# arneschneuing/DiffSBDD

Measured on AMD Instinct MI355X. Metric: sampled ligands/sec (500-step DDPM, fullatom_cond) at 1/2/4/8 MI355X, higher is better.
Workload: dtype f32

## Files before the change

diffsbdd_amd/csrc/edge_mlp.h:

```cpp
#pragma once
#include "common.h"

namespace dsbdd {

struct EdgeMlpW {
  const float* P;
  const float* Q;
  const float* wd;
  const float* wd0;
  const float* table;
  const float* W2T;
  const float* b2;
  const float* W2TP;
  const float* W2TP16;
  const void* W2E;
  const float* W2SK;
};

__global__ void permute_w2t_kernel(const float* src, float* dst, int H) {
  const int i = blockIdx.x * blockDim.x + threadIdx.x;
  if (i >= H * H) return;
  const int k = i / H, o = i % H, ct = H / 32;
  const int j = o / ct, c = o % ct;
  dst[i] = src[k * H + c * 32 + j];
// ... 62 lines not shown
  const int row = (blockIdx.x * kThreads + threadIdx.x) >> 6, lane = threadIdx.x & 63;
  if (row >= n_rows + n_ghost) return;
  const bool ghost = row >= n_rows;
  const int da = ghost ? 0 : deg_a[row], sa = ghost ? 0 : row_ptr_a[row];
  const int a0 = sa >> 5, a1 = min((sa + da - 1) >> 5, max_tile);
  int db = 0, sb = 0, tw = 0;
  if (row >= n_lig) {
    const int tl = ghost ? row - n_rows : twin_local[row - n_lig];
    db = deg_b[tl]; sb = row_ptr_b[tl]; tw = twin_base + tl;
  }
  const int b0 = sb >> 5, b1 = min((sb + db - 1) >> 5, max_tile);
  for (int k = 4 * lane; k < H; k += 256) {
    float4 v = make_float4(0.f, 0.f, 0.f, 0.f);
    if (da > 0) {
      v = ld4(agg + (size_t)row * H + k);
      for (int T = a0 + 1; T <= a1; ++T) {
        const float4 h = ld4(head_a + (size_t)T * H + k);
        v.x += h.x; v.y += h.y; v.z += h.z; v.w += h.w;
      }
    }
    if (db > 0) {
      float4 u = ld4(agg_b + (size_t)tw * H + k);
      for (int T = b0 + 1; T <= b1; ++T) {
        const float4 h = ld4(head_b + (size_t)T * H + k);
        u.x += h.x; u.y += h.y; u.z += h.z; u.w += h.w;
      }
      v.x += u.x; v.y += u.y; v.z += u.z; v.w += u.w;
    }
    *reinterpret_cast<float4*>(agg + (size_t)row * H + k) = v;
  }
}


__global__ __launch_bounds__(kThreads) void agg_complete_shell_kernel(
    float* agg, const float* agg_head, const int* row_ptr, const int* deg, int n_rows, int H, int max_tile,
    const int* lvl, int shell_level, int n_lig, int n_nodes, const float* head_s, const int* sh_ptr, const int* sh_deg,
    const int* row_ptr_nat, const int* ecol_nat, int e_cap_nat, const int* twin_local, const int* row_ptr_ghost,
    const float* msg, int msg_slots, float inv_norm) {
  const int row = (blockIdx.x * kThreads + threadIdx.x) >> 6, lane = threadIdx.x & 63;
  if (row >= n_rows) return;
  const int L = (row >= n_lig && row < n_nodes) ? lvl[row] : 0;
  if (L > shell_level) return;
  if (L < shell_level) {
    const int d = deg[row], s = row_ptr[row];
    const int t0 = s >> 5, t1 = min((s + d - 1) >> 5, max_tile);
    if (d > 0 && t1 == t0) return;
    for (int k = 4 * lane; k < H; k += 256) {
      float4 v = make_float4(0.f, 0.f, 0.f, 0.f);
      if (d > 0) {
        v = ld4(agg + (size_t)row * H + k);
        for (int T = t0 + 1; T <= t1; ++T) {
          const float4 h = ld4(agg_head + (size_t)T * H + k);
          v.x += h.x; v.y += h.y; v.z += h.z; v.w += h.w;
        }
      }
      *reinterpret_cast<float4*>(agg + (size_t)row * H + k) = v;
    }
    return;
  }
  const int d = sh_deg[row], s = sh_ptr[row];
  const int t0 = s >> 5, t1 = min((s + d - 1) >> 5, max_tile);
  const int dn = deg[row], sn = row_ptr_nat[row];
  const int e_lo = max(sn, 0), e_hi = min(sn + dn, e_cap_nat);
  const int base = row_ptr_ghost[twin_local[row - n_lig]] - sn;
  const int k = min(4 * lane, H - 4);
  const bool on = 4 * lane < H;
  float4 v = make_float4(0.f, 0.f, 0.f, 0.f);
  if (d > 0 && on) {
    v = ld4(agg + (size_t)row * H + k);
    for (int T = t0 + 1; T <= t1; ++T) {
      const float4 h = ld4(head_s + (size_t)T * H + k);
      v.x += h.x; v.y += h.y; v.z += h.z; v.w += h.w;
    }
  }
  float4 c = make_float4(0.f, 0.f, 0.f, 0.f);
  for (int e0 = e_lo; e0 < e_hi; e0 += 64) {
    const int e = e0 + lane;
    bool take = false;
    if (e < e_hi) {
      const int j = ecol_nat[e];
      take = (unsigned)j < (unsigned)n_nodes && j >= n_lig && lvl[j] >= shell_level &&
             (unsigned)(base + e) < (unsigned)msg_slots;
    }
    unsigned long long mk = __ballot(take);
    while (mk) {
      const float* src[4];
      int n = 0;
#pragma unroll
      for (int u = 0; u < 4; ++u)
        if (mk) {
          src[n++] = msg + (size_t)(base + e0 + (__ffsll((long long)mk) - 1)) * H + k;
          mk &= mk - 1;
        }
      float4 m[4];
#pragma unroll
      for (int u = 0; u < 4; ++u) if (u < n) m[u] = ld4(src[u]);
#pragma unroll
      for (int u = 0; u < 4; ++u) if (u < n) { c.x += m[u].x; c.y += m[u].y; c.z += m[u].z; c.w += m[u].w; }
    }
  }
  v.x += c.x * inv_norm; v.y += c.y * inv_norm; v.z += c.z * inv_norm; v.w += c.w * inv_norm;
  if (on) *reinterpret_cast<float4*>(agg + (size_t)row * H + k) = v;
}

}
```

diffsbdd_amd/csrc/engine.hip:

```cpp
#include "../../include/diffsbdd_hip.h"

#include <algorithm>
#include <climits>
#include <cmath>
#include <cstdio>
#include <cstdlib>
#include <cstring>
#include <string>
#include <type_traits>
#include <utility>
#include <vector>

#include "common.h"
#include "ddpm.h"
#include "edge_mlp.h"
#include "edge_wave.h"
#include "edge_wave16.h"
#include "edge_splitk.h"
#include "graph_parts.h"
#include "radius_graph.h"
#include "level_list.h"
#include "geometry.h"
#include "lig_head.h"
#include "ligand_pack.h"
// ... 229 lines not shown
  double tot = 0.0;
  for (size_t i = 0; i + 1 < e->ev_used; i += 2) {
    HIP_TRY(hipEventSynchronize(e->ev[i + 1]));
    float ms = 0.f;
    HIP_TRY(hipEventElapsedTime(&ms, e->ev[i], e->ev[i + 1]));
    tot += ms;
  }
  *total_ms = tot;
  *launches = (int64_t)(e->ev_used / 2);
  e->ev_used = 0;
  return DSBDD_OK;
}

int dsbdd_engine_graph_stats(const dsbdd_engine* e, int64_t* replays, int64_t* captures, int64_t* eager) {
  if (!e || !replays || !captures || !eager) return fail(DSBDD_ERR_ARG, "null argument");
  *replays = e->n_replay; *captures = e->n_capture; *eager = e->n_eager;
  return DSBDD_OK;
}

int dsbdd_engine_buffer(const dsbdd_engine* e, int which, void** out) {
  if (!e || !out || !e->ws) return fail(DSBDD_ERR_STATE, "no workspace bound");
  void* const buf[] = {e->erow, e->ecol, e->ed0, e->row_ptr, e->h, e->x, e->node_batch, e->deg, e->lvl, e->lvl_list, e->lvl_cnt,
                       e->lvl_end, e->row_ptrL, e->erowL, e->ecolL, e->ed0L, e->lvl_stats};
  static_assert(DSBDD_BUF_LEVEL_STATS + 1 == sizeof(buf) / sizeof(buf[0]), "one pointer per DSBDD_BUF_* id");
  if (which < 0 || which > DSBDD_BUF_LEVEL_STATS) return fail(DSBDD_ERR_ARG, "unknown buffer id");
  *out = buf[which];
  return DSBDD_OK;
}

int dsbdd_engine_list2_read(const dsbdd_engine* e, int which, void* dst, int64_t count) {
  if (!e || !dst || count < 0) return fail(DSBDD_ERR_ARG, "bad argument");
  if (!e->ws) return fail(DSBDD_ERR_STATE, "no workspace bound");
  const int64_t N = e->cap_lig + e->cap_poc;
  const int* src = which == DSBDD_LIST2_DEG ? e->deg2 : (which == DSBDD_LIST2_ROW_PTR ? e->row_ptr2 : nullptr);
  if (!src) return fail(DSBDD_ERR_ARG, "unknown list-2 buffer");
  if (count > N + (which == DSBDD_LIST2_ROW_PTR ? 1 : 0)) return fail(DSBDD_ERR_CAPACITY, "list-2 read past the buffer");
  HIP_TRY(hipDeviceSynchronize());
  HIP_TRY(hipMemcpy(dst, src, (size_t)count * 4, hipMemcpyDeviceToHost));
  return DSBDD_OK;
}

int dsbdd_engine_shell_read(const dsbdd_engine* e, int which, int list, void* dst, int64_t count) {
  if (!e || !dst || count < 0) return fail(DSBDD_ERR_ARG, "bad argument");
  if (!e->shell_mem) return fail(DSBDD_ERR_STATE, "no shell stage has run on this engine");
  const int64_t N = e->shell_key[0], SL = e->shell_key[2];
  const void* src = nullptr;
  int64_t have = 0, size = 4;
  const bool lst = list >= 0 && list < kShellLists;
  switch (which) {
    case DSBDD_SHELL_STATS: src = e->sh_stats; have = 8; size = 8; break;
    case DSBDD_SHELL_COUNT: src = e->sh_cnt; have = kShellLists; break;
    case DSBDD_SHELL_ROW: if (lst) { src = e->sh_row + (size_t)list * SL; have = SL; } break;
    case DSBDD_SHELL_COL: if (lst) { src = e->sh_col + (size_t)list * SL; have = SL; } break;
    case DSBDD_SHELL_PTR: src = e->sh_ptr; have = N; break;
    case DSBDD_SHELL_DEG: src = e->sh_deg; have = N; break;
  }
  if (!src) return fail(DSBDD_ERR_ARG, "unknown shell buffer");
  if (count > have) return fail(DSBDD_ERR_CAPACITY, "shell read past the buffer");
  HIP_TRY(hipDeviceSynchronize());
  HIP_TRY(hipMemcpy(dst, src, (size_t)(count * size), hipMemcpyDeviceToHost));
  return DSBDD_OK;
}

int dsbdd_dynamics_forward(dsbdd_engine* e, void* stream, const float* xh_lig, const float* xh_pocket,
                           const float* t, int64_t t_count, const int64_t* mask_lig,
                           const int64_t* mask_pocket, int64_t n_lig, int64_t n_pocket, int64_t batch,
                           const int32_t* ext_row, const int32_t* ext_col, int64_t ext_n_edges,
                           float* eps_lig, float* eps_pocket, int32_t* status) {
  StreamDevice stream_device_(stream);
  if (!e || !xh_lig || !xh_pocket || !t || !mask_lig || !mask_pocket || !eps_lig || !status)
    return fail(DSBDD_ERR_ARG, "null argument");
  if (!e->has_weights) return fail(DSBDD_ERR_STATE, "weights not set");
  if (!e->ws) return fail(DSBDD_ERR_STATE, "workspace not bound");
  if (n_lig > e->cap_lig || n_pocket > e->cap_poc || batch > e->cap_batch || n_lig < 0 || n_pocket < 0 ||
      batch < 1)
    return fail(DSBDD_ERR_CAPACITY, "sizes exceed the bound workspace");
  if (t_count != 1 && t_count != batch) return fail(DSBDD_ERR_ARG, "t must have 1 or batch entries");
  if (ext_row && (!ext_col || ext_n_edges < 0 || ext_n_edges > e->cap_edges))
    return fail(DSBDD_ERR_CAPACITY, "external edge list exceeds edge capacity");
  hipStream_t s = static_cast<hipStream_t>(stream);
  const ForwardArgs args{xh_lig, xh_pocket, t, t_count, mask_lig, mask_pocket, n_lig, n_pocket, batch,
                         ext_row, ext_col, ext_n_edges, eps_lig, eps_pocket, status};
  const int rc = frame_upkeep(e, s, args);
  if (rc) return rc;
  e->time_now = e->profile > 0 && (e->prof_call++ % e->profile) == 0;
  if (!e->use_graph || e->time_now || e->trace_h || e->trace_x || ext_row) {
    ++e->n_eager;
    return forward_impl(e, s, args);
// ... 6 lines not shown
```

diffsbdd_amd/csrc/graph_parts.h:

```cpp
#pragma once
#include "common.h"

namespace dsbdd {

constexpr int kTileCtrInts = 32;
constexpr int kEdgeAlign = 32;
constexpr int kLevels = 5;
constexpr int kShellLists = 2;

__host__ __device__ __forceinline__ int align_edges(int v) { return (v + kEdgeAlign - 1) & ~(kEdgeAlign - 1); }

template <class I>
__device__ __forceinline__ int lower_bound_i64(const I* a, int n, long long v) {
  static_assert(sizeof(I) == 8, "64-bit masks");
  int lo = 0, hi = n;
  while (lo < hi) {
    const int mid = (lo + hi) >> 1;
    if (a[mid] < v) lo = mid + 1; else hi = mid;
  }
  return lo;
}

struct SampleRows {
  int l0, l1, p0, p1;
// ... 65 lines not shown
    const int idx = lo + lane * step;
    const int c = __popcll(__ballot(idx < hi && a[idx] < v));
    if (c == 0) return lo;
    const int last = lo + (c - 1) * step;
    hi = min(last + step, hi);
    lo = last + 1;
  }
  return lo;
}

__device__ __forceinline__ SampleRows sample_rows_wg(const int64_t* mask_lig, int n_lig, const int64_t* mask_poc,
                                                     int n_poc, int b, int* s_rows) {
  static_assert(kThreads == 256, "one wave per bound");
  const int w = threadIdx.x >> 6, lane = threadIdx.x & 63;
  const int r = w < 2 ? lower_bound_wave(mask_lig, n_lig, b + (w & 1), lane)
                      : lower_bound_wave(mask_poc, n_poc, b + (w & 1), lane);
  if (lane == 0) s_rows[w] = r;
  __syncthreads();
  return SampleRows{s_rows[0], s_rows[1], s_rows[2], s_rows[3]};
}

__device__ __forceinline__ void sample_mean_body(const float* x, const int* lig_off, const int* poc_off, int n_lig,
                                                 float* mean, float (*red)[kThreads]) {
  const int b = blockIdx.x, t = threadIdx.x;
  const SampleRows r = sample_rows(lig_off, poc_off, n_lig, b);
  float s0 = 0.f, s1 = 0.f, s2 = 0.f;
  for (int i = r.l0 + t; i < r.l1; i += kThreads) { s0 += x[3 * i]; s1 += x[3 * i + 1]; s2 += x[3 * i + 2]; }
  for (int i = r.p0 + t; i < r.p1; i += kThreads) { s0 += x[3 * i]; s1 += x[3 * i + 1]; s2 += x[3 * i + 2]; }
  block_sum3(s0, s1, s2, red);
  if (t < 3) mean[3 * b + t] = red[t][0] / (float)r.count();
  __syncthreads();
}

__device__ __forceinline__ int pad_fill(int from, int lane, int* erow, int* ecol, float* ed0, int cap) {
  const int to = align_edges(from), pos = from + lane;
  if (pos >= 0 && pos < to && pos < cap) { erow[pos] = -1; ecol[pos] = 0; ed0[pos] = 0.f; }
  return to;
}

__global__ void zero_kernel(uint4* p, size_t n16, unsigned char* tail, int n_tail) {
  const uint4 z = make_uint4(0u, 0u, 0u, 0u);
  for (size_t i = blockIdx.x * (size_t)blockDim.x + threadIdx.x; i < n16; i += (size_t)gridDim.x * blockDim.x)
    p[i] = z;
  if (blockIdx.x == 0 && (int)threadIdx.x < n_tail) tail[threadIdx.x] = 0;
}

inline hipError_t zero_async(void* ptr, size_t bytes, hipStream_t s) {
  if (bytes == 0) return hipSuccess;
  const size_t n16 = bytes / 16;
  const int n_tail = (int)(bytes % 16);
  size_t blocks = (n16 + 255) / 256;
  if (blocks > 2048) blocks = 2048;
  if (blocks < 1) blocks = 1;
  hipLaunchKernelGGL(zero_kernel, dim3((unsigned)blocks), dim3(256), 0, s, static_cast<uint4*>(ptr), n16,
                     static_cast<unsigned char*>(ptr) + n16 * 16, n_tail);
  return hipGetLastError();
}

}
```

diffsbdd_amd/csrc/launch.h:

```cpp
#pragma once

static hipError_t nl(hipStream_t s, const float* A1, int lda1, int K1, const float* A2, int lda2, int K2,
                     const float* WT, int ldw, const float* bias, const float* R, int ldr, float* C,
                     int ldc, int64_t M, int N, int act) {
  NodeLinearArgs a{A1, lda1, K1, A2, lda2, K2, WT, ldw, bias, R, ldr, C, ldc, (int)M, N, act, nullptr, nullptr};
  return launch_node_linear(s, a);
}

template <class... P, class... A>
static int launch_1d(void (*kernel)(P...), size_t n_items, hipStream_t s, A... args) {
  hipLaunchKernelGGL(kernel, dim3((unsigned)((n_items + 255) / 256)), dim3(256), 0, s, static_cast<P>(args)...);
  HIP_TRY(hipGetLastError());
  return DSBDD_OK;
}

static int device_cus() {
  static int cache[64] = {0};
  int dev = 0;
  if (hipGetDevice(&dev) != hipSuccess || dev < 0 || dev >= 64) return 256;
  if (cache[dev] == 0) {
    hipDeviceProp_t pr;
    int n = 0;
    if (hipGetDeviceProperties(&pr, dev) == hipSuccess) n = pr.multiProcessorCount;
    cache[dev] = n > 0 ? n : 256;
// ... 88 lines not shown
    a.tail_s = e->tail > 1 ? e->tail : resident;
    grid = persistent_grid((edge_bound + 127) / 128 * 4, e->n_cu, 2, e->edge_max_wg, 8);
  }
  if (a.msg_out) {
    if (mode != MODE_GCL || e->cfg.hidden_nf != 256 || e->emu || !a.mlp[0].W2TP || a.wt_base) return hipErrorInvalidValue;
    hipLaunchKernelGGL((edge_wave_kernel<256, MODE_GCL, true, 0, false, true>), dim3(grid), dim3(kThreads), 0, s, a);
    return hipGetLastError();
  }
  return with_hidden(e->cfg.hidden_nf, [&](auto h) {
    constexpr int H = decltype(h)::value;
    return emu ? launch_wave_emu_t<H>(s, mode, a, grid, emu) : launch_wave_t<H>(s, mode, a, grid);
  });
}

static hipError_t launch_edge_plain(int H, hipStream_t s, int mode, const EdgeArgs& a, int64_t edge_bound) {
  const int grid = edge_wave_grid(mode, a, edge_bound, device_cus(), 0);
  if (a.z2_out && (a.e_count_b || a.wt_base)) return hipErrorInvalidValue;
  return with_hidden(H, [&](auto h) {
    constexpr int HH = decltype(h)::value;
    return a.z2_out ? launch_wave_store_t<HH>(s, mode, a, grid) : launch_wave_t<HH>(s, mode, a, grid);
  });
}

static Cutoffs cutoffs_of(const dsbdd_config& c) {
  return Cutoffs{c.has_cutoff_ligand, c.has_cutoff_pocket, c.has_cutoff_interaction,
                 c.cutoff_ligand, c.cutoff_pocket, c.cutoff_interaction};
}

static int build_edges_impl(hipStream_t s, const float* x, int n_lig, int N, int B, const dsbdd_config& c,
                            const int* node_batch, const int* lig_off, const int* poc_off, int* deg,
                            int* row_ptr, int* erow, int* ecol, float* ed0, int64_t cap, int* status,
                            int* act_flag = nullptr, int* scan_tmp = nullptr, int* seg_base = nullptr,
                            const EdgeList2* list2 = nullptr, int id_offset = 0, int* lvl = nullptr) {
  const int waves_per_block = kThreads / 64;
  int blocks = (N + waves_per_block - 1) / waves_per_block;
  if (blocks > 4096) blocks = 4096;
  if (blocks < 1) blocks = 1;
  const Cutoffs cut = cutoffs_of(c);
  const int aligned = scan_tmp && seg_base;
  SegAlign sg{node_batch, lig_off, poc_off, n_lig, B, scan_tmp, aligned ? seg_base : nullptr};
  EdgeList2 l2{};
  if (list2 && aligned) l2 = *list2;
  hipLaunchKernelGGL((edges_kernel<false>), dim3(blocks), dim3(kThreads), 0, s, x, node_batch, lig_off,
                     poc_off, n_lig, N, cut, deg, (const int*)nullptr, (int*)nullptr, (int*)nullptr,
                     (float*)nullptr, 0, status, act_flag, SegAlign{}, (int*)nullptr, l2, 0, lvl);
  HIP_TRY(hipGetLastError());
  hipLaunchKernelGGL(scan_kernel, dim3(l2.deg ? 2 : 1), dim3(1024), 0, s, (const int*)deg, row_ptr, N, sg,
                     (const int*)l2.deg, l2.row_ptr, l2.seg);
  HIP_TRY(hipGetLastError());
  hipLaunchKernelGGL((edges_kernel<true>), dim3(blocks), dim3(kThreads), 0, s, x, node_batch, lig_off,
                     poc_off, n_lig, N, cut, deg, (const int*)row_ptr, erow, ecol, ed0, (int)cap, status,
                     (int*)nullptr, sg, row_ptr, l2, id_offset, (int*)nullptr);
  HIP_TRY(hipGetLastError());
  return DSBDD_OK;
}
```

diffsbdd_amd/csrc/level_list.h:

```cpp
#pragma once
#include "common.h"
#include "graph_parts.h"

namespace dsbdd {

struct LevelArgs {
  const int* node_batch; const int* lig_off; const int* poc_off; int n_lig; int B;
  int* lvl;
  const int* deg;
  const int* row_ptr_nat;
  const int* erow_nat; const int* ecol_nat; const float* ed0_nat;
  int* seg_rows;
  int* seg_edges;
  int* node_base;
  int* edge_base;
  int* lvl_cnt;
  int* lvl_end;
  int* lvl_list;
  int* row_ptr;
  int* erow; int* ecol; float* ed0; int e_cap;
  unsigned long long* stats;
  int node_off; int edge_off;
  int e_cap_nat;
  const float* mean_x; float* mean_out;
// ... 268 lines not shown
    const int incl = wave_scan_incl(d, lane);
    if (mine) {
      a.lvl_list[n_run + __popcll(m & ((1ull << lane) - 1ull))] = i;
      a.row_ptr[i] = e_run + incl - d;
    }
    n_run += __popcll(m);
    e_run += __shfl(incl, 63);
    if (shell) {
      const int d2 = mine ? a.sh_deg[i] : 0;
      const int incl2 = wave_scan_incl(d2, lane);
      if (mine) a.sh_ptr[i] = s_run + incl2 - d2;
      s_run += __shfl(incl2, 63);
    }
  }
  pad_fill(e_run, lane, a.erow, a.ecol, a.ed0, a.e_cap);
  if (shell) {
    const size_t o = (size_t)sl * a.sh_cap;
    const int to = pad_fill(s_run, lane, a.sh_row + o, a.sh_col + o, a.sh_d0 + o, a.sh_cap);
    if (lane == 0) {
      if (b == a.B - 1) a.sh_cnt[sl] = to;
      if (a.sh_stats) {
        const int own = s_run - s_begin;
        atomicAdd(&a.sh_stats[3 * sl], (unsigned long long)own);
        atomicAdd(&a.sh_stats[3 * sl + 1], (unsigned long long)(to - s_begin));
        atomicAdd(&a.sh_stats[3 * sl + 2], (unsigned long long)(a.seg_edges[L * a.B + b] - own));
        if (b == 0 && sl == 0) atomicAdd(&a.sh_stats[3 * kShellLists], 1ull);
      }
    }
  }
}

__global__ void level_copy_kernel(LevelArgs a, int n_nodes) {
  const int total = min(a.row_ptr_nat[n_nodes], a.e_cap_nat);
  for (int e = blockIdx.x * blockDim.x + threadIdx.x; e < total; e += gridDim.x * blockDim.x) {
    const int i = a.erow_nat[e];
    if (i < 0 || i >= n_nodes) continue;
    const int pos = a.row_ptr[i] + (e - a.row_ptr_nat[i]);
    if (pos >= 0 && pos < a.e_cap) { a.erow[pos] = i; a.ecol[pos] = a.ecol_nat[e]; a.ed0[pos] = a.ed0_nat[e]; }
    const int L = i >= a.n_lig ? a.lvl[i] : 0;
    if (L >= 2 && L - 2 < a.n_shell) {
      const int j = a.ecol_nat[e];
      if (j < a.n_lig || a.lvl[j] < L) {
        int rank = 0;
        for (int q = max(a.row_ptr_nat[i], 0); q < e; ++q) {
          const int jq = a.ecol_nat[q];
          rank += (jq < a.n_lig || a.lvl[jq] < L) ? 1 : 0;
        }
        const int ps = a.sh_ptr[i] + rank;
        const size_t o = (size_t)(L - 2) * a.sh_cap;
        if (ps >= 0 && ps < a.sh_cap) { a.sh_row[o + ps] = i; a.sh_col[o + ps] = j; a.sh_d0[o + ps] = a.ed0_nat[e]; }
      }
    }
  }
}

__global__ void ghost_setup_kernel(const int* erow3, const int* ecol3, const float* ed03, const int* row_ptr3,
                                   const int* deg3, int n3, int id_src, int id_dst, int* erow, int* ecol,
                                   float* ed0, int e_cap, int* deg, int* row_ptr, int* lvl_list,
                                   const float* xframe, float* x) {
  const int total = min(row_ptr3[n3], e_cap);
  for (int p = blockIdx.x * blockDim.x + threadIdx.x; p < total; p += gridDim.x * blockDim.x) {
    const int r = erow3[p];
    erow[p] = r < 0 ? -1 : r - id_src + id_dst;
    ecol[p] = r < 0 ? 0 : ecol3[p] - id_src + id_dst;
    ed0[p] = ed03[p];
  }
  for (int i = blockIdx.x * blockDim.x + threadIdx.x; i < n3; i += gridDim.x * blockDim.x) {
    deg[id_dst + i] = deg3[i];
    row_ptr[id_dst + i] = row_ptr3[i];
    lvl_list[i] = id_dst + i;
    x[3 * (id_dst + i)] = xframe[3 * i]; x[3 * (id_dst + i) + 1] = xframe[3 * i + 1];
    x[3 * (id_dst + i) + 2] = xframe[3 * i + 2];
  }
}

__global__ __launch_bounds__(kThreads) void gather_rows_kernel(float* dst, const float* src, const int* rows, int n,
                                                               int H) {
  const int i = (blockIdx.x * kThreads + threadIdx.x) >> 6, lane = threadIdx.x & 63;
  if (i >= n) return;
  const float* a = src + (size_t)rows[i] * H;
  float* b = dst + (size_t)i * H;
  for (int k = 4 * lane; k < H; k += 256) *reinterpret_cast<float4*>(b + k) = ld4(a + k);
}

// ... 18 lines not shown
```

diffsbdd_amd/csrc/radius_graph.h:

```cpp
#pragma once
#include "common.h"
#include "graph_parts.h"

namespace dsbdd {

struct Cutoffs {
  int has_l, has_p, has_i;
  float cl, cp, ci;
};

__device__ __forceinline__ void prep_offsets(int i, const int64_t* mask_lig, int n_lig, const int64_t* mask_poc,
                                             int n_poc, int B, int* lig_off, int* poc_off, int* tile_ctr) {
  if (tile_ctr && i < kTileCtrInts) tile_ctr[i] = 0;
  if (i <= B) {
    lig_off[i] = lower_bound_i64(mask_lig, n_lig, i);
    poc_off[i] = lower_bound_i64(mask_poc, n_poc, i);
  }
}
__device__ __forceinline__ int prep_node(int i, const int64_t* mask_lig, int n_lig, const int64_t* mask_poc,
                                         int* node_batch) {
  const int b = (int)(i < n_lig ? mask_lig[i] : mask_poc[i - n_lig]);
  node_batch[i] = b;
  return b;
}

__global__ void prep_kernel(const int64_t* mask_lig, int n_lig, const int64_t* mask_poc, int n_poc,
                            int B, int* node_batch, int* lig_off, int* poc_off, int* tile_ctr) {
  const int i = blockIdx.x * blockDim.x + threadIdx.x;
  prep_offsets(i, mask_lig, n_lig, mask_poc, n_poc, B, lig_off, poc_off, tile_ctr);
  if (i < n_lig + n_poc) prep_node(i, mask_lig, n_lig, mask_poc, node_batch);
}

struct SegAlign {
  const int* node_batch; const int* lig_off; const int* poc_off;
  int n_lig; int B;
  int* scan_tmp;
  int* seg_base;
};

struct EdgeList2 {
  int* deg; int* row_ptr; int* erow; int* ecol; float* ed0; int e_cap;
  SegAlign seg;
};

template <bool FILL>
__global__ __launch_bounds__(kThreads) void edges_kernel(
    const float* __restrict__ x, const int* __restrict__ node_batch,
    const int* __restrict__ lig_off, const int* __restrict__ poc_off, int n_lig, int n_nodes,
    Cutoffs cut, int* __restrict__ deg, const int* __restrict__ row_ptr, int* __restrict__ erow,
    int* __restrict__ ecol, float* __restrict__ ed0, int e_cap, int* __restrict__ status,
    int* __restrict__ act_flag, SegAlign seg, int* __restrict__ row_ptr_out, EdgeList2 l2, int id_offset,
    int* __restrict__ lvl = nullptr) {
  const int lane = threadIdx.x & 63;
  const int wave = (blockIdx.x * blockDim.x + threadIdx.x) >> 6;
  const int nwaves = (gridDim.x * blockDim.x) >> 6;
  for (int i = wave; i < n_nodes; i += nwaves) {
    const int b = node_batch[i];
    const bool il = i < n_lig;
    const float xi = x[3 * i], yi = x[3 * i + 1], zi = x[3 * i + 2];
    int base = 0;
    int base2 = 0;
    if (FILL) {
      if (seg.seg_base) {
        const int k = il ? b : seg.B + b;
        const int first = il ? lig_off[b] : n_lig + poc_off[b];
        base = seg.seg_base[k] + seg.scan_tmp[i] - seg.scan_tmp[first];
        if (lane == 0) row_ptr_out[i] = base;
      } else {
        base = row_ptr[i];
      }
    }
    if (FILL && l2.deg) {
      const int k = il ? b : l2.seg.B + b;
      const int first = il ? lig_off[b] : n_lig + poc_off[b];
      base2 = l2.seg.seg_base[k] + l2.seg.scan_tmp[i] - l2.seg.scan_tmp[first];
      if (lane == 0) l2.row_ptr[i] = base2;
    }
    int cnt = 0, cnt_lig = 0;
#pragma unroll 1
    for (int seg = 0; seg < 2; ++seg) {
      const int j_begin = seg == 0 ? lig_off[b] : n_lig + poc_off[b];
      const int j_end = seg == 0 ? lig_off[b + 1] : n_lig + poc_off[b + 1];
      const bool jl = seg == 0;
      const int has = (il && jl) ? cut.has_l : ((!il && !jl) ? cut.has_p : cut.has_i);
      const float c = (il && jl) ? cut.cl : ((!il && !jl) ? cut.cp : cut.ci);
      for (int j0 = j_begin; j0 < j_end; j0 += 64) {
        const int j = j0 + lane;
        const bool valid = j < j_end;
        float d2 = 0.f;
        if (valid) {
          const float dx = xi - x[3 * j], dy = yi - x[3 * j + 1], dz = zi - x[3 * j + 2];
          d2 = dx * dx + dy * dy + dz * dz;
        }
        const bool pass = valid && (!has || __fsqrt_rn(d2) <= c);
        const unsigned long long m = __ballot(pass);
        if (FILL && pass) {
          const int pos = base + cnt + __popcll(m & ((1ull << lane) - 1ull));
          if (pos >= 0 && pos < e_cap) {
            erow[pos] = i + id_offset; ecol[pos] = j + id_offset; ed0[pos] = d2;
          }
          if (l2.deg && (il || jl)) {
            const int pos2 = base2 + cnt + __popcll(m & ((1ull << lane) - 1ull));
            if (pos2 >= 0 && pos2 < l2.e_cap) { l2.erow[pos2] = i; l2.ecol[pos2] = j; l2.ed0[pos2] = d2; }
          }
        }
        cnt += __popcll(m);
      }
      if (seg == 0) cnt_lig = cnt;
    }
    if (!FILL && lane == 0) {
      deg[i] = cnt;
      if (l2.deg) l2.deg[i] = il ? cnt : cnt_lig;
      if (act_flag) act_flag[i] = (il || cnt_lig > 0) ? 1 : 0;
      if (lvl) lvl[i] = il ? 0 : (cnt_lig > 0 ? 1 : kLevels - 1);
    }
    if (FILL && lane == 0 && base + cnt > e_cap) atomicOr(status, 2);
    if (FILL && seg.seg_base) {
      const int seg_last = (il ? lig_off[b + 1] : n_lig + poc_off[b + 1]) - 1;
      if (i == seg_last) {
        pad_fill(base + cnt, lane, erow, ecol, ed0, e_cap);
        if (l2.deg) pad_fill(base2 + (il ? cnt : cnt_lig), lane, l2.erow, l2.ecol, l2.ed0, l2.e_cap);
      }
    }
  }
}

__device__ void scan_one(const int* deg, int* row_ptr, int n, SegAlign seg, int* s_wave, int* s_carry_p);

__global__ __launch_bounds__(1024) void scan_kernel(const int* deg, int* row_ptr, int n, SegAlign seg,
                                                    const int* deg_b, int* row_ptr_b, SegAlign seg_b) {
  __shared__ int s_wave[16];
  __shared__ int s_carry;
  if (blockIdx.x == 0) scan_one(deg, row_ptr, n, seg, s_wave, &s_carry);
  else if (deg_b) scan_one(deg_b, row_ptr_b, n, seg_b, s_wave, &s_carry);
}

__device__ void scan_one(const int* deg, int* row_ptr, int n, SegAlign seg, int* s_wave, int* s_carry_p) {
  int& s_carry = *s_carry_p;
  const int t = threadIdx.x;
  int* out = seg.seg_base ? seg.scan_tmp : row_ptr;
  const bool vec = ((reinterpret_cast<uintptr_t>(deg) | reinterpret_cast<uintptr_t>(out)) & 15) == 0;
  int carry = 0;
  for (int base = 0; base < n; base += 4096) {
    const int i0 = base + 4 * t;
    int v[4] = {0, 0, 0, 0};
    if (vec && i0 + 3 < n) {
      const int4 q = *reinterpret_cast<const int4*>(deg + i0);
      v[0] = q.x; v[1] = q.y; v[2] = q.z; v[3] = q.w;
    } else {
#pragma unroll
      for (int k = 0; k < 4; ++k) if (i0 + k < n) v[k] = deg[i0 + k];
    }
    const int mine = v[0] + v[1] + v[2] + v[3];
    int run = carry + block_scan_1024(mine, s_wave, s_carry_p);
    const int tile_total = s_carry;
// ... 59 lines not shown
```

include/diffsbdd_hip.h:

```cpp
#ifndef DIFFSBDD_HIP_H
#define DIFFSBDD_HIP_H

#include <stddef.h>
#include <stdint.h>

#ifdef __cplusplus
extern "C" {
#endif

#define DSBDD_ABI_VERSION 6

enum {
  DSBDD_OK = 0,
  DSBDD_ERR_ARG = -1,
  DSBDD_ERR_STATE = -2,
  DSBDD_ERR_CAPACITY = -3,
  DSBDD_ERR_LAUNCH = -4
};

enum {
  DSBDD_STATUS_NAN = 1,
  DSBDD_STATUS_EDGE_OVERFLOW = 2
};

// ... 65 lines not shown
int dsbdd_engine_clear_pocket_frame(dsbdd_engine* e);

int dsbdd_engine_set_trace(dsbdd_engine* e, float* trace_h, float* trace_x);

int dsbdd_dynamics_forward(dsbdd_engine* e, void* stream, const float* xh_lig,
                           const float* xh_pocket, const float* t, int64_t t_count,
                           const int64_t* mask_lig, const int64_t* mask_pocket, int64_t n_lig,
                           int64_t n_pocket, int64_t batch, const int32_t* ext_row,
                           const int32_t* ext_col, int64_t ext_n_edges, float* eps_lig,
                           float* eps_pocket, int32_t* status);

int dsbdd_engine_profile(dsbdd_engine* e, int enable, int max_launches);
int dsbdd_engine_profile_read(dsbdd_engine* e, double* total_ms, int64_t* launches);

int dsbdd_engine_graph_stats(const dsbdd_engine* e, int64_t* replays, int64_t* captures, int64_t* eager);

int dsbdd_engine_last_plan(const dsbdd_engine* e, int32_t* radius, int32_t* ghost, int32_t capacity,
                           int32_t* n_stages, int32_t* timed_level);

enum { DSBDD_OPT_PRUNE = 0, DSBDD_OPT_CONE = 1, DSBDD_OPT_GRANULE16 = 2, DSBDD_OPT_EMU = 3, DSBDD_OPT_SPLITK = 4,
       DSBDD_OPT_SHELL = 5, DSBDD_OPT_TAIL = 6 };
int dsbdd_engine_set_option(dsbdd_engine* e, int which, int value);
int dsbdd_engine_get_option(const dsbdd_engine* e, int which);

enum {
  DSBDD_BUF_EDGE_ROW = 0, DSBDD_BUF_EDGE_COL, DSBDD_BUF_EDGE_D0, DSBDD_BUF_ROW_PTR,
  DSBDD_BUF_H, DSBDD_BUF_X, DSBDD_BUF_NODE_BATCH, DSBDD_BUF_DEG,
  DSBDD_BUF_LEVEL, DSBDD_BUF_LEVEL_LIST, DSBDD_BUF_LEVEL_COUNT, DSBDD_BUF_LEVEL_END,
  DSBDD_BUF_LROW_PTR, DSBDD_BUF_LEDGE_ROW, DSBDD_BUF_LEDGE_COL, DSBDD_BUF_LEDGE_D0,
  DSBDD_BUF_LEVEL_STATS
};
int dsbdd_engine_buffer(const dsbdd_engine* e, int which, void** ptr_out);

enum { DSBDD_SHELL_STATS = 0, DSBDD_SHELL_COUNT, DSBDD_SHELL_ROW, DSBDD_SHELL_COL, DSBDD_SHELL_PTR, DSBDD_SHELL_DEG };
int dsbdd_engine_shell_read(const dsbdd_engine* e, int which, int list, void* dst, int64_t count);

enum { DSBDD_LIST2_DEG = 0, DSBDD_LIST2_ROW_PTR };
int dsbdd_engine_list2_read(const dsbdd_engine* e, int which, void* dst, int64_t count);

int dsbdd_cond_reverse_update(void* stream, float* z_lig, float* xh_pocket, const float* eps_lig,
                              const float* noise, const int64_t* mask_lig,
                              const int64_t* mask_pocket, int64_t n_lig, int64_t n_pocket,
                              int64_t batch, int32_t atom_nf, int32_t residue_nf, float alpha_ts,
                              float c_eps, float sigma, int32_t remove_com);

int dsbdd_joint_reverse_update(void* stream, float* z_lig, float* z_pocket, const float* eps_lig,
                               const float* eps_pocket, const float* noise_lig,
                               const float* noise_pocket, const int64_t* mask_lig,
                               const int64_t* mask_pocket, int64_t n_lig, int64_t n_pocket,
                               int64_t batch, int32_t atom_nf, int32_t residue_nf, float alpha_ts,
                               float c_eps, float sigma, int32_t center_noise);

int dsbdd_segment_mean3(void* stream, const float* x, int32_t ld, const int64_t* mask, int64_t n_rows,
                        int64_t batch, float* out);

int dsbdd_cond_affine_noise(void* stream, float* z_lig, float* xh_pocket, const float* noise,
                            const int64_t* mask_lig, const int64_t* mask_pocket, int64_t n_lig,
                            int64_t n_pocket, int64_t batch, int32_t atom_nf, int32_t residue_nf, float a,
                            float sigma, int32_t remove_com);

int dsbdd_joint_affine_noise(void* stream, float* z_lig, float* z_pocket, const float* noise_lig,
                             const float* noise_pocket, const int64_t* mask_lig, const int64_t* mask_pocket,
                             int64_t n_lig, int64_t n_pocket, int64_t batch, int32_t atom_nf,
                             int32_t residue_nf, float a, float sigma, int32_t center_noise,
                             int32_t remove_com);

int dsbdd_cond_repaint_update(void* stream, float* z_lig, float* xh_pocket, float* scratch_lig,
                              const float* xh0_lig, const float* com_pocket0, const float* fixed,
                              const float* noise_known, const float* noise_resample, const int64_t* mask_lig,
                              const int64_t* mask_pocket, int64_t n_lig, int64_t n_pocket, int64_t batch,
// ... 229 lines not shown
```

Baseline: 42.11.

## Restructure radius-graph, shell-copy and shell aggregation kernels for fewer serial loads

The edge-building kernel now runs a 2D grid, one batch sample per y-block, and stages that sample's coordinates in shared memory so each row is processed without scattered global reads. The shell level-copy kernel replaces a per-thread serial rank loop with wave ballots and popcounts. The shell aggregation kernel hoists its per-row index loads and keeps up to 8 message loads in flight instead of 4. Debug read-back accessors for list-2 and shell d0 buffers are also added. The aim is to cut latency-bound graph-construction and aggregation overhead, at the cost of more LDS use, extra registers and more complex indexing.

After: 42.30, median of 6. About the same (+0.5%).

```diff
diff --git a/diffsbdd_amd/csrc/edge_mlp.h b/diffsbdd_amd/csrc/edge_mlp.h
--- a/diffsbdd_amd/csrc/edge_mlp.h
+++ b/diffsbdd_amd/csrc/edge_mlp.h
@@ -118,6 +118,7 @@
 }
 
 
+constexpr int kShellInFlight = 8;
 __global__ __launch_bounds__(kThreads) void agg_complete_shell_kernel(
     float* agg, const float* agg_head, const int* row_ptr, const int* deg, int n_rows, int H, int max_tile,
     const int* lvl, int shell_level, int n_lig, int n_nodes, const float* head_s, const int* sh_ptr, const int* sh_deg,
@@ -125,10 +126,14 @@
     const float* msg, int msg_slots, float inv_norm) {
   const int row = (blockIdx.x * kThreads + threadIdx.x) >> 6, lane = threadIdx.x & 63;
   if (row >= n_rows) return;
-  const int L = (row >= n_lig && row < n_nodes) ? lvl[row] : 0;
+  const bool pocket = row >= n_lig && row < n_nodes;
+  const int pr = pocket ? row : n_lig;
+  const int L_ld = lvl[pr], deg_r = deg[row], ptr_r = row_ptr[row];
+  const int shd = sh_deg[pr], shp = sh_ptr[pr], sn_ld = row_ptr_nat[pr], tw = twin_local[pr - n_lig];
+  const int L = pocket ? L_ld : 0;
   if (L > shell_level) return;
   if (L < shell_level) {
-    const int d = deg[row], s = row_ptr[row];
+    const int d = deg_r, s = ptr_r;
     const int t0 = s >> 5, t1 = min((s + d - 1) >> 5, max_tile);
     if (d > 0 && t1 == t0) return;
     for (int k = 4 * lane; k < H; k += 256) {
@@ -144,11 +149,15 @@
     }
     return;
   }
-  const int d = sh_deg[row], s = sh_ptr[row];
+  const int d = shd, s = shp;
   const int t0 = s >> 5, t1 = min((s + d - 1) >> 5, max_tile);
-  const int dn = deg[row], sn = row_ptr_nat[row];
+  const int dn = deg_r, sn = sn_ld;
   const int e_lo = max(sn, 0), e_hi = min(sn + dn, e_cap_nat);
-  const int base = row_ptr_ghost[twin_local[row - n_lig]] - sn;
+  int j_first = -1;
+  if (e_lo + lane < e_hi) j_first = ecol_nat[e_lo + lane];
+  const bool j_ok = (unsigned)j_first < (unsigned)n_nodes && j_first >= n_lig;
+  const int lj_first = j_ok ? lvl[j_first] : -1;
+  const int base = row_ptr_ghost[tw] - sn;
   const int k = min(4 * lane, H - 4);
   const bool on = 4 * lane < H;
   float4 v = make_float4(0.f, 0.f, 0.f, 0.f);
@@ -164,25 +173,30 @@
     const int e = e0 + lane;
     bool take = false;
     if (e < e_hi) {
-      const int j = ecol_nat[e];
-      take = (unsigned)j < (unsigned)n_nodes && j >= n_lig && lvl[j] >= shell_level &&
+      int lj = lj_first;
+      if (e0 != e_lo) {
+        const int j = ecol_nat[e];
+        lj = ((unsigned)j < (unsigned)n_nodes && j >= n_lig) ? lvl[j] : -1;
+      }
+      take = lj >= shell_level &&
              (unsigned)(base + e) < (unsigned)msg_slots;
     }
     unsigned long long mk = __ballot(take);
     while (mk) {
-      const float* src[4];
-      int n = 0;
+      const float* src[kShellInFlight];
+      bool has[kShellInFlight];
 #pragma unroll
-      for (int u = 0; u < 4; ++u)
-        if (mk) {
-          src[n++] = msg + (size_t)(base + e0 + (__ffsll((long long)mk) - 1)) * H + k;
-          mk &= mk - 1;
-        }
-      float4 m[4];
+      for (int u = 0; u < kShellInFlight; ++u) {
+        has[u] = mk != 0;
+        src[u] = msg + (size_t)(base + e0 + (has[u] ? __ffsll((long long)mk) - 1 : 0)) * H + k;
+        mk &= mk - 1;
+      }
+      float4 m[kShellInFlight];
 #pragma unroll
-      for (int u = 0; u < 4; ++u) if (u < n) m[u] = ld4(src[u]);
+      for (int u = 0; u < kShellInFlight; ++u) if (has[u]) m[u] = ld4(src[u]);
 #pragma unroll
-      for (int u = 0; u < 4; ++u) if (u < n) { c.x += m[u].x; c.y += m[u].y; c.z += m[u].z; c.w += m[u].w; }
+      for (int u = 0; u < kShellInFlight; ++u)
+        if (has[u]) { c.x += m[u].x; c.y += m[u].y; c.z += m[u].z; c.w += m[u].w; }
     }
   }
   v.x += c.x * inv_norm; v.y += c.y * inv_norm; v.z += c.z * inv_norm; v.w += c.w * inv_norm;
diff --git a/diffsbdd_amd/csrc/engine.hip b/diffsbdd_amd/csrc/engine.hip
--- a/diffsbdd_amd/csrc/engine.hip
+++ b/diffsbdd_amd/csrc/engine.hip
@@ -285,9 +285,18 @@
   if (!e || !dst || count < 0) return fail(DSBDD_ERR_ARG, "bad argument");
   if (!e->ws) return fail(DSBDD_ERR_STATE, "no workspace bound");
   const int64_t N = e->cap_lig + e->cap_poc;
-  const int* src = which == DSBDD_LIST2_DEG ? e->deg2 : (which == DSBDD_LIST2_ROW_PTR ? e->row_ptr2 : nullptr);
+  const void* src = nullptr;
+  int64_t have = 0;
+  switch (which) {
+    case DSBDD_LIST2_DEG: src = e->deg2; have = N; break;
+    case DSBDD_LIST2_ROW_PTR: src = e->row_ptr2; have = N + 1; break;
+    case DSBDD_LIST2_ROW: src = e->erow2; have = e->cap_edges; break;
+    case DSBDD_LIST2_COL: src = e->ecol2; have = e->cap_edges; break;
+    case DSBDD_LIST2_D0: src = e->ed02; have = e->cap_edges; break;
+    case DSBDD_LIST2_ACT: src = e->act_flag; have = N; break;
+  }
   if (!src) return fail(DSBDD_ERR_ARG, "unknown list-2 buffer");
-  if (count > N + (which == DSBDD_LIST2_ROW_PTR ? 1 : 0)) return fail(DSBDD_ERR_CAPACITY, "list-2 read past the buffer");
+  if (count > have) return fail(DSBDD_ERR_CAPACITY, "list-2 read past the buffer");
   HIP_TRY(hipDeviceSynchronize());
   HIP_TRY(hipMemcpy(dst, src, (size_t)count * 4, hipMemcpyDeviceToHost));
   return DSBDD_OK;
@@ -307,6 +316,7 @@
     case DSBDD_SHELL_COL: if (lst) { src = e->sh_col + (size_t)list * SL; have = SL; } break;
     case DSBDD_SHELL_PTR: src = e->sh_ptr; have = N; break;
     case DSBDD_SHELL_DEG: src = e->sh_deg; have = N; break;
+    case DSBDD_SHELL_D0: if (lst) { src = e->sh_d0 + (size_t)list * SL; have = SL; } break;
   }
   if (!src) return fail(DSBDD_ERR_ARG, "unknown shell buffer");
   if (count > have) return fail(DSBDD_ERR_CAPACITY, "shell read past the buffer");
diff --git a/diffsbdd_amd/csrc/graph_parts.h b/diffsbdd_amd/csrc/graph_parts.h
--- a/diffsbdd_amd/csrc/graph_parts.h
+++ b/diffsbdd_amd/csrc/graph_parts.h
@@ -121,6 +121,11 @@
   __syncthreads();
 }
 
+__device__ __forceinline__ float pair_d2(float xi, float yi, float zi, float xj, float yj, float zj) {
+  const float dx = xi - xj, dy = yi - yj, dz = zi - zj;
+  return dx * dx + dy * dy + dz * dz;
+}
+
 __device__ __forceinline__ int pad_fill(int from, int lane, int* erow, int* ecol, float* ed0, int cap) {
   const int to = align_edges(from), pos = from + lane;
   if (pos >= 0 && pos < to && pos < cap) { erow[pos] = -1; ecol[pos] = 0; ed0[pos] = 0.f; }
diff --git a/diffsbdd_amd/csrc/launch.h b/diffsbdd_amd/csrc/launch.h
--- a/diffsbdd_amd/csrc/launch.h
+++ b/diffsbdd_amd/csrc/launch.h
@@ -144,24 +144,28 @@
                             int* row_ptr, int* erow, int* ecol, float* ed0, int64_t cap, int* status,
                             int* act_flag = nullptr, int* scan_tmp = nullptr, int* seg_base = nullptr,
                             const EdgeList2* list2 = nullptr, int id_offset = 0, int* lvl = nullptr) {
-  const int waves_per_block = kThreads / 64;
-  int blocks = (N + waves_per_block - 1) / waves_per_block;
-  if (blocks > 4096) blocks = 4096;
-  if (blocks < 1) blocks = 1;
+  auto grid_for = [&](int rows_per_wave) {
+    const int rows_per_block = (kThreads / 64) * rows_per_wave;
+    const int avg = (N + B - 1) / B;
+    int slices = (avg + rows_per_block - 1) / rows_per_block;
+    if (slices > 8192 / B) slices = 8192 / B;
+    if (slices < 1) slices = 1;
+    return dim3(slices, B < 65535 ? B : 65535);
+  };
   const Cutoffs cut = cutoffs_of(c);
   const int aligned = scan_tmp && seg_base;
   SegAlign sg{node_batch, lig_off, poc_off, n_lig, B, scan_tmp, aligned ? seg_base : nullptr};
   EdgeList2 l2{};
   if (list2 && aligned) l2 = *list2;
-  hipLaunchKernelGGL((edges_kernel<false>), dim3(blocks), dim3(kThreads), 0, s, x, node_batch, lig_off,
-                     poc_off, n_lig, N, cut, deg, (const int*)nullptr, (int*)nullptr, (int*)nullptr,
+  hipLaunchKernelGGL((edges_kernel<false>), grid_for(kEdgeRowsCount), dim3(kThreads), 0, s, x, lig_off,
+                     poc_off, n_lig, B, cut, deg, (const int*)nullptr, (int*)nullptr, (int*)nullptr,
                      (float*)nullptr, 0, status, act_flag, SegAlign{}, (int*)nullptr, l2, 0, lvl);
   HIP_TRY(hipGetLastError());
   hipLaunchKernelGGL(scan_kernel, dim3(l2.deg ? 2 : 1), dim3(1024), 0, s, (const int*)deg, row_ptr, N, sg,
                      (const int*)l2.deg, l2.row_ptr, l2.seg);
   HIP_TRY(hipGetLastError());
-  hipLaunchKernelGGL((edges_kernel<true>), dim3(blocks), dim3(kThreads), 0, s, x, node_batch, lig_off,
-                     poc_off, n_lig, N, cut, deg, (const int*)row_ptr, erow, ecol, ed0, (int)cap, status,
+  hipLaunchKernelGGL((edges_kernel<true>), grid_for(kEdgeRowsFill), dim3(kThreads), 0, s, x, lig_off,
+                     poc_off, n_lig, B, cut, deg, (const int*)row_ptr, erow, ecol, ed0, (int)cap, status,
                      (int*)nullptr, sg, row_ptr, l2, id_offset, (int*)nullptr);
   HIP_TRY(hipGetLastError());
   return DSBDD_OK;
diff --git a/diffsbdd_amd/csrc/level_list.h b/diffsbdd_amd/csrc/level_list.h
--- a/diffsbdd_amd/csrc/level_list.h
+++ b/diffsbdd_amd/csrc/level_list.h
@@ -324,24 +324,45 @@
 
 __global__ void level_copy_kernel(LevelArgs a, int n_nodes) {
   const int total = min(a.row_ptr_nat[n_nodes], a.e_cap_nat);
-  for (int e = blockIdx.x * blockDim.x + threadIdx.x; e < total; e += gridDim.x * blockDim.x) {
-    const int i = a.erow_nat[e];
-    if (i < 0 || i >= n_nodes) continue;
-    const int pos = a.row_ptr[i] + (e - a.row_ptr_nat[i]);
-    if (pos >= 0 && pos < a.e_cap) { a.erow[pos] = i; a.ecol[pos] = a.ecol_nat[e]; a.ed0[pos] = a.ed0_nat[e]; }
-    const int L = i >= a.n_lig ? a.lvl[i] : 0;
-    if (L >= 2 && L - 2 < a.n_shell) {
-      const int j = a.ecol_nat[e];
-      if (j < a.n_lig || a.lvl[j] < L) {
-        int rank = 0;
-        for (int q = max(a.row_ptr_nat[i], 0); q < e; ++q) {
+  const int lane = threadIdx.x & 63;
+  for (int e = blockIdx.x * blockDim.x + threadIdx.x; e - lane < total; e += gridDim.x * blockDim.x) {
+    const int e0 = e - lane;
+    const bool in = e < total;
+    const int i = in ? a.erow_nat[e] : -1;
+    const int j = in ? a.ecol_nat[e] : 0;
+    const float d0 = in ? a.ed0_nat[e] : 0.f;
+    const bool row_ok = i >= 0 && i < n_nodes;
+    const int s_nat = row_ok ? a.row_ptr_nat[i] : 0;
+    const int L = (row_ok && i >= a.n_lig) ? a.lvl[i] : 0;
+    if (row_ok) {
+      const int pos = a.row_ptr[i] + (e - s_nat);
+      if (pos >= 0 && pos < a.e_cap) { a.erow[pos] = i; a.ecol[pos] = j; a.ed0[pos] = d0; }
+    }
+    if (a.n_shell <= 0) continue;
+    const bool shell = L >= 2 && L - 2 < a.n_shell;
+    const int sp = shell ? a.sh_ptr[i] : 0;
+    const bool mine = shell && (j < a.n_lig || a.lvl[j] < L);
+    const unsigned long long m = __ballot(mine);
+    const int i_first = __shfl(i, 0), s_first = max(__shfl(s_nat, 0), 0), L_first = __shfl(L, 0);
+    int carry = 0;
+    if (i_first >= 0 && i_first < n_nodes && L_first >= 2 && L_first - 2 < a.n_shell)
+      for (int q0 = e0 - 64; q0 + 64 > s_first; q0 -= 64) {
+        const int q = q0 + lane;
+        bool f = false;
+        if (q >= s_first) {
           const int jq = a.ecol_nat[q];
-          rank += (jq < a.n_lig || a.lvl[jq] < L) ? 1 : 0;
+          f = jq < a.n_lig || a.lvl[jq] < L_first;
         }
-        const int ps = a.sh_ptr[i] + rank;
-        const size_t o = (size_t)(L - 2) * a.sh_cap;
-        if (ps >= 0 && ps < a.sh_cap) { a.sh_row[o + ps] = i; a.sh_col[o + ps] = j; a.sh_d0[o + ps] = a.ed0_nat[e]; }
-      }
+        carry += __popcll(__ballot(f));
+      }
+    if (mine) {
+      const int lo = max(s_nat, 0) - e0;
+      const unsigned long long below = (1ull << lane) - 1ull;
+      const unsigned long long own = lo > 0 ? below & ~((1ull << lo) - 1ull) : below;
+      const int rank = __popcll(m & own) + (lo < 0 ? carry : 0);
+      const int ps = sp + rank;
+      const size_t o = (size_t)(L - 2) * a.sh_cap;
+      if (ps >= 0 && ps < a.sh_cap) { a.sh_row[o + ps] = i; a.sh_col[o + ps] = j; a.sh_d0[o + ps] = d0; }
     }
   }
 }
diff --git a/diffsbdd_amd/csrc/radius_graph.h b/diffsbdd_amd/csrc/radius_graph.h
--- a/diffsbdd_amd/csrc/radius_graph.h
+++ b/diffsbdd_amd/csrc/radius_graph.h
@@ -43,84 +43,116 @@
   SegAlign seg;
 };
 
+constexpr int kEdgeNodes = 512;
+constexpr int kEdgeRowsCount = 3, kEdgeRowsFill = 4;
+
+template <bool FILL, bool LDS>
+__device__ __forceinline__ void edges_row(
+    const int i, const int b, const SampleRows& r, const float* __restrict__ s_x, const float* __restrict__ x,
+    const int n_lig, const Cutoffs& cut, int* __restrict__ deg, const int* __restrict__ row_ptr,
+    int* __restrict__ erow, int* __restrict__ ecol, float* __restrict__ ed0, const int e_cap, int* __restrict__ status,
+    int* __restrict__ act_flag, const SegAlign& seg, int* __restrict__ row_ptr_out, const EdgeList2& l2,
+    const int id_offset, int* __restrict__ lvl) {
+  const int lane = threadIdx.x & 63;
+  const int nl = r.l1 - r.l0;
+  const bool il = i < n_lig;
+  const int ci = il ? i - r.l0 : nl + (i - r.p0);
+  const float xi = LDS ? s_x[3 * ci] : x[3 * i], yi = LDS ? s_x[3 * ci + 1] : x[3 * i + 1],
+              zi = LDS ? s_x[3 * ci + 2] : x[3 * i + 2];
+  int base = 0;
+  int base2 = 0;
+  if (FILL) {
+    if (seg.seg_base) {
+      const int k = il ? b : seg.B + b;
+      const int first = il ? r.l0 : r.p0;
+      base = seg.seg_base[k] + seg.scan_tmp[i] - seg.scan_tmp[first];
+      if (lane == 0) row_ptr_out[i] = base;
+    } else {
+      base = row_ptr[i];
+    }
+  }
+  if (FILL && l2.deg) {
+    const int k = il ? b : l2.seg.B + b;
+    const int first = il ? r.l0 : r.p0;
+    base2 = l2.seg.seg_base[k] + l2.seg.scan_tmp[i] - l2.seg.scan_tmp[first];
+    if (lane == 0) l2.row_ptr[i] = base2;
+  }
+  int cnt = 0, cnt_lig = 0;
+#pragma unroll 1
+  for (int sg = 0; sg < 2; ++sg) {
+    const int j_begin = sg == 0 ? r.l0 : r.p0;
+    const int j_end = sg == 0 ? r.l1 : r.p1;
+    const int c_begin = sg == 0 ? 0 : nl;
+    const bool jl = sg == 0;
+    const int has = (il && jl) ? cut.has_l : ((!il && !jl) ? cut.has_p : cut.has_i);
+    const float c = (il && jl) ? cut.cl : ((!il && !jl) ? cut.cp : cut.ci);
+    for (int j0 = j_begin; j0 < j_end; j0 += 64) {
+      const int j = j0 + lane;
+      const bool valid = j < j_end;
+      float d2 = 0.f;
+      if (valid) {
+        const int cj = c_begin + (j - j_begin);
+        d2 = LDS ? pair_d2(xi, yi, zi, s_x[3 * cj], s_x[3 * cj + 1], s_x[3 * cj + 2])
+                 : pair_d2(xi, yi, zi, x[3 * j], x[3 * j + 1], x[3 * j + 2]);
+      }
+      const bool pass = valid && (!has || __fsqrt_rn(d2) <= c);
+      const unsigned long long m = __ballot(pass);
+      if (FILL && pass) {
+        const int pos = base + cnt + __popcll(m & ((1ull << lane) - 1ull));
+        if (pos >= 0 && pos < e_cap) {
+          erow[pos] = i + id_offset; ecol[pos] = j + id_offset; ed0[pos] = d2;
+        }
+        if (l2.deg && (il || jl)) {
+          const int pos2 = base2 + cnt + __popcll(m & ((1ull << lane) - 1ull));
+          if (pos2 >= 0 && pos2 < l2.e_cap) { l2.erow[pos2] = i; l2.ecol[pos2] = j; l2.ed0[pos2] = d2; }
+        }
+      }
+      cnt += __popcll(m);
+    }
+    if (sg == 0) cnt_lig = cnt;
+  }
+  if (!FILL && lane == 0) {
+    deg[i] = cnt;
+    if (l2.deg) l2.deg[i] = il ? cnt : cnt_lig;
+    if (act_flag) act_flag[i] = (il || cnt_lig > 0) ? 1 : 0;
+    if (lvl) lvl[i] = il ? 0 : (cnt_lig > 0 ? 1 : kLevels - 1);
+  }
+  if (FILL && lane == 0 && base + cnt > e_cap) atomicOr(status, 2);
+  if (FILL && seg.seg_base) {
+    const int seg_last = (il ? r.l1 : r.p1) - 1;
+    if (i == seg_last) {
+      pad_fill(base + cnt, lane, erow, ecol, ed0, e_cap);
+      if (l2.deg) pad_fill(base2 + (il ? cnt : cnt_lig), lane, l2.erow, l2.ecol, l2.ed0, l2.e_cap);
+    }
+  }
+}
+
 template <bool FILL>
 __global__ __launch_bounds__(kThreads) void edges_kernel(
-    const float* __restrict__ x, const int* __restrict__ node_batch,
-    const int* __restrict__ lig_off, const int* __restrict__ poc_off, int n_lig, int n_nodes,
+    const float* __restrict__ x, const int* __restrict__ lig_off, const int* __restrict__ poc_off, int n_lig, int B,
     Cutoffs cut, int* __restrict__ deg, const int* __restrict__ row_ptr, int* __restrict__ erow,
     int* __restrict__ ecol, float* __restrict__ ed0, int e_cap, int* __restrict__ status,
     int* __restrict__ act_flag, SegAlign seg, int* __restrict__ row_ptr_out, EdgeList2 l2, int id_offset,
     int* __restrict__ lvl = nullptr) {
-  const int lane = threadIdx.x & 63;
-  const int wave = (blockIdx.x * blockDim.x + threadIdx.x) >> 6;
-  const int nwaves = (gridDim.x * blockDim.x) >> 6;
-  for (int i = wave; i < n_nodes; i += nwaves) {
-    const int b = node_batch[i];
-    const bool il = i < n_lig;
-    const float xi = x[3 * i], yi = x[3 * i + 1], zi = x[3 * i + 2];
-    int base = 0;
-    int base2 = 0;
-    if (FILL) {
-      if (seg.seg_base) {
-        const int k = il ? b : seg.B + b;
-        const int first = il ? lig_off[b] : n_lig + poc_off[b];
-        base = seg.seg_base[k] + seg.scan_tmp[i] - seg.scan_tmp[first];
-        if (lane == 0) row_ptr_out[i] = base;
-      } else {
-        base = row_ptr[i];
-      }
-    }
-    if (FILL && l2.deg) {
-      const int k = il ? b : l2.seg.B + b;
-      const int first = il ? lig_off[b] : n_lig + poc_off[b];
-      base2 = l2.seg.seg_base[k] + l2.seg.scan_tmp[i] - l2.seg.scan_tmp[first];
-      if (lane == 0) l2.row_ptr[i] = base2;
-    }
-    int cnt = 0, cnt_lig = 0;
-#pragma unroll 1
-    for (int seg = 0; seg < 2; ++seg) {
-      const int j_begin = seg == 0 ? lig_off[b] : n_lig + poc_off[b];
-      const int j_end = seg == 0 ? lig_off[b + 1] : n_lig + poc_off[b + 1];
-      const bool jl = seg == 0;
-      const int has = (il && jl) ? cut.has_l : ((!il && !jl) ? cut.has_p : cut.has_i);
-      const float c = (il && jl) ? cut.cl : ((!il && !jl) ? cut.cp : cut.ci);
-      for (int j0 = j_begin; j0 < j_end; j0 += 64) {
-        const int j = j0 + lane;
-        const bool valid = j < j_end;
-        float d2 = 0.f;
-        if (valid) {
-          const float dx = xi - x[3 * j], dy = yi - x[3 * j + 1], dz = zi - x[3 * j + 2];
-          d2 = dx * dx + dy * dy + dz * dz;
-        }
-        const bool pass = valid && (!has || __fsqrt_rn(d2) <= c);
-        const unsigned long long m = __ballot(pass);
-        if (FILL && pass) {
-          const int pos = base + cnt + __popcll(m & ((1ull << lane) - 1ull));
-          if (pos >= 0 && pos < e_cap) {
-            erow[pos] = i + id_offset; ecol[pos] = j + id_offset; ed0[pos] = d2;
-          }
-          if (l2.deg && (il || jl)) {
-            const int pos2 = base2 + cnt + __popcll(m & ((1ull << lane) - 1ull));
-            if (pos2 >= 0 && pos2 < l2.e_cap) { l2.erow[pos2] = i; l2.ecol[pos2] = j; l2.ed0[pos2] = d2; }
-          }
-        }
-        cnt += __popcll(m);
-      }
-      if (seg == 0) cnt_lig = cnt;
-    }
-    if (!FILL && lane == 0) {
-      deg[i] = cnt;
-      if (l2.deg) l2.deg[i] = il ? cnt : cnt_lig;
-      if (act_flag) act_flag[i] = (il || cnt_lig > 0) ? 1 : 0;
-      if (lvl) lvl[i] = il ? 0 : (cnt_lig > 0 ? 1 : kLevels - 1);
-    }
-    if (FILL && lane == 0 && base + cnt > e_cap) atomicOr(status, 2);
-    if (FILL && seg.seg_base) {
-      const int seg_last = (il ? lig_off[b + 1] : n_lig + poc_off[b + 1]) - 1;
-      if (i == seg_last) {
-        pad_fill(base + cnt, lane, erow, ecol, ed0, e_cap);
-        if (l2.deg) pad_fill(base2 + (il ? cnt : cnt_lig), lane, l2.erow, l2.ecol, l2.ed0, l2.e_cap);
-      }
+  __shared__ float s_x[3 * kEdgeNodes];
+  const int t = threadIdx.x;
+  const int w0 = blockIdx.x * (kThreads / 64) + (t >> 6), nw = gridDim.x * (kThreads / 64);
+  for (int b = blockIdx.y; b < B; b += gridDim.y) {
+    const SampleRows r = sample_rows(lig_off, poc_off, n_lig, b);
+    const int nl = r.l1 - r.l0, np = r.p1 - r.p0, nn = nl + np;
+    if ((int)blockIdx.x * (kThreads / 64) >= nn) continue;
+    if (nl >= 0 && np >= 0 && nn <= kEdgeNodes) {
+      for (int q = t; q < 3 * nl; q += kThreads) s_x[q] = x[3 * r.l0 + q];
+      for (int q = t; q < 3 * np; q += kThreads) s_x[3 * nl + q] = x[3 * r.p0 + q];
+      __syncthreads();
+      for (int k = w0; k < nn; k += nw)
+        edges_row<FILL, true>(k < nl ? r.l0 + k : r.p0 + (k - nl), b, r, s_x, x, n_lig, cut, deg, row_ptr, erow, ecol,
+                              ed0, e_cap, status, act_flag, seg, row_ptr_out, l2, id_offset, lvl);
+      __syncthreads();
+    } else {
+      for (int k = w0; k < nn; k += nw)
+        edges_row<FILL, false>(k < nl ? r.l0 + k : r.p0 + (k - nl), b, r, s_x, x, n_lig, cut, deg, row_ptr, erow, ecol,
+                               ed0, e_cap, status, act_flag, seg, row_ptr_out, l2, id_offset, lvl);
     }
   }
 }
diff --git a/include/diffsbdd_hip.h b/include/diffsbdd_hip.h
--- a/include/diffsbdd_hip.h
+++ b/include/diffsbdd_hip.h
@@ -121,10 +121,11 @@
 };
 int dsbdd_engine_buffer(const dsbdd_engine* e, int which, void** ptr_out);
 
-enum { DSBDD_SHELL_STATS = 0, DSBDD_SHELL_COUNT, DSBDD_SHELL_ROW, DSBDD_SHELL_COL, DSBDD_SHELL_PTR, DSBDD_SHELL_DEG };
+enum { DSBDD_SHELL_STATS = 0, DSBDD_SHELL_COUNT, DSBDD_SHELL_ROW, DSBDD_SHELL_COL, DSBDD_SHELL_PTR, DSBDD_SHELL_DEG,
+       DSBDD_SHELL_D0 };
 int dsbdd_engine_shell_read(const dsbdd_engine* e, int which, int list, void* dst, int64_t count);
 
-enum { DSBDD_LIST2_DEG = 0, DSBDD_LIST2_ROW_PTR };
+enum { DSBDD_LIST2_DEG = 0, DSBDD_LIST2_ROW_PTR, DSBDD_LIST2_ROW, DSBDD_LIST2_COL, DSBDD_LIST2_D0, DSBDD_LIST2_ACT };
 int dsbdd_engine_list2_read(const dsbdd_engine* e, int which, void* dst, int64_t count);
 
 int dsbdd_cond_reverse_update(void* stream, float* z_lig, float* xh_pocket, const float* eps_lig,
```
